# stegben/neural-locality-sensitive-hashing

Hardware: AMD Instinct MI355X
Metric: queries/sec + recall@10, SIFT1M 128-d 16-bit hash, 1/2/4/8 GPU (higher is better)
Workload: dtype f32

## Files before the change

include/nlsh_hip.h:

```cpp
#ifndef NLSH_HIP_H
#define NLSH_HIP_H

#include <stddef.h>
#include <stdint.h>

#ifdef __cplusplus
extern "C" {
#endif

#define NLSH_ABI_VERSION 4

typedef void *nlsh_stream_t;

enum {
    NLSH_OK = 0,
    NLSH_E_INVALID = -1,
    NLSH_E_UNSUPPORTED = -2,
    NLSH_E_HIP = -3,
    NLSH_E_WORKSPACE = -4
};

enum { NLSH_ACT_SIGMOID = 0, NLSH_ACT_TANH = 1 };
enum { NLSH_KEY_REF_INT16 = 0, NLSH_KEY_FULL = 1 };
enum { NLSH_METRIC_L2_EPS = 0, NLSH_METRIC_COSINE = 1, NLSH_METRIC_L2_EPS_FOLDED = 2 };
// ... 206 lines not shown
    int64_t Q;
    int32_t *qkeys, *nkeys;
    float *out_dist;
    int32_t *out_idx;
    uint64_t *out_keys;
    int32_t *out_ncand, *status;
    void *workspace;
    size_t workspace_bytes;
    int64_t max_tasks;
    nlsh_stream_t front, plan, mid, tail;
} nlsh_step_desc_t;

int nlsh_step_create(const nlsh_step_desc_t *desc, size_t desc_bytes, nlsh_step_t **step_out);
int nlsh_step_create_graph(const nlsh_step_desc_t *desc, size_t desc_bytes, nlsh_stream_t lane, nlsh_step_t **step_out);
int nlsh_step_destroy(nlsh_step_t *step);
int nlsh_step_set_weights(nlsh_step_t *step, const float *packed);
int nlsh_query_step_enqueue(nlsh_step_t *step, const float *queries, int64_t q_stride, uint64_t seed, nlsh_stream_t producer,
                            void *ev_scan_begin, void *ev_scan_end);
int nlsh_step_release(nlsh_step_t *step);
int nlsh_query_batch(const nlsh_step_desc_t *desc, size_t desc_bytes, const float *queries, int64_t q_stride, uint64_t seed,
                     int64_t row0, int lookup_done, void *ev_scan_begin, void *ev_scan_end, nlsh_stream_t stream);
int nlsh_query_batch_host(const nlsh_step_desc_t *desc, size_t desc_bytes, const float *queries, int64_t q_stride, uint64_t seed,
                          int64_t row0, int lookup_done, int32_t *host_out, size_t host_words, nlsh_stream_t stream);
size_t nlsh_query_batch_ranked_scratch(int64_t Q, int H);
int nlsh_query_batch_ranked(const nlsh_step_desc_t *desc, size_t desc_bytes, const float *queries, int64_t q_stride, int lookup_done,
                            int32_t budget, void *scratch, size_t scratch_bytes, int32_t *host_out, size_t host_words,
                            void *ev_scan_begin, void *ev_scan_end, nlsh_stream_t stream);
int nlsh_step_busy(nlsh_step_t *step);

int nlsh_merge_topk(const uint64_t *keys_in, int64_t row_stride, int G, int64_t Q, int k, const int32_t *ncand_in,
                    float *out_dist, int32_t *out_idx, int32_t *out_ncand, nlsh_stream_t stream);

#define NLSH_MAX_TABLES 16
int nlsh_merge_topk_unique(const uint64_t *keys_in, int64_t row_stride, int G, int64_t Q, int k, const int32_t *ncand_in,
                           float *out_dist, int32_t *out_idx, uint64_t *out_keys , int32_t *out_ncand, nlsh_stream_t stream);

#define NLSH_EXACT_L2 0
#define NLSH_EXACT_COSINE 1
size_t nlsh_exact_workspace(int64_t Q, int64_t N, int k, int splits);
int nlsh_exact_topk(const float *corpus, int64_t row_stride, int64_t N, int d,
                    const float *queries, int64_t q_stride, int64_t Q, int k, int metric,
                    int64_t self_row0 , int splits ,
                    float *out_dist, int32_t *out_idx, void *workspace, size_t workspace_bytes, nlsh_stream_t stream);

#ifdef __cplusplus
}
// ... 3 lines not shown
```

neural-locality-sensitive-hashing_amd/csrc/step.hip:

```cpp
#include <cstdlib>
#include <new>

#include "step_nodes.h"

#include "scan_bucket_args.h"

using namespace nlsh;

struct nlsh_step {
    EncPlan enc;
    nlsh_step_desc_t d;
    int dims[NLSH_MAX_LAYERS + 1];
    hipEvent_t ready, encoded, planned, scanned, done;
    bool done_pending;
    hipStream_t lane;
    hipGraph_t graph;
    hipGraphExec_t exec;
    hipGraphNode_t enc_node, scan_node;
    bool graph_failed;
};

static BucketScanCall step_scan_call(const nlsh_step_desc_t &d, const float *queries, int64_t q_stride, hipStream_t stream, int phases) {
    BucketScanCall c = {};
    c.corpus = d.corpus_sorted; c.row_stride = d.row_stride; c.d = d.d; c.gid = d.gid; c.uniq = d.uniq_keys; c.offsets = d.offsets;
    c.bucket_order = d.bucket_order; c.nb = d.n_buckets; c.cell_of = d.cell_of; c.cell_offsets = d.cell_offsets; c.n_cells = d.n_cells;
    c.inv_norm = d.inv_norm; c.queries = queries; c.q_stride = q_stride; c.Q = d.Q; c.qkeys = d.qkeys; c.nkeys = d.nkeys;
    c.P = d.n_probes; c.k = d.k; c.metric = d.metric; c.algo = d.algo; c.seg = d.seg_rows;
    c.out_dist = d.out_dist; c.out_idx = d.out_idx; c.out_keys = d.out_keys; c.out_ncand = d.out_ncand; c.status = d.status;
    c.workspace = d.workspace; c.workspace_bytes = d.workspace_bytes; c.max_tasks = d.max_tasks;
    c.stream = stream; c.phases = phases;
    return c;
}
constexpr int SCAN_AND_MERGE = NLSH_PHASE_SCAN | NLSH_PHASE_MERGE;
static int step_scan_check(const BucketScanCall &c) { return scan_call_check("scan_topk", c, SCAN_NEEDS_TOPK_OUT | SCAN_ALLOWS_PLAN_REST); }
static int step_scan_prepare(const BucketScanCall &c, BucketScanPrep *p) {
    const int rc = step_scan_check(c);
    return rc != NLSH_OK ? rc : bucket_scan_args(c, p);
}
static int step_scan_run(const BucketScanCall &c) {
    const int rc = step_scan_check(c);
    if (rc != NLSH_OK || c.Q == 0) return rc;
    return scan_call_run(c);
// ... 23 lines not shown
static int step_create(const nlsh_step_desc_t *desc, size_t desc_bytes, hipStream_t lane, nlsh_step_t **out) {
    NLSH_REQUIRE(desc && out, NLSH_E_INVALID, "step_create: null pointer");
    NLSH_REQUIRE(desc_bytes == sizeof(nlsh_step_desc_t), NLSH_E_INVALID, "step_create: descriptor of %zu bytes, this library's is %zu (ABI %d)",
                 desc_bytes, sizeof(nlsh_step_desc_t), NLSH_ABI_VERSION);
    if (lane == nullptr) {
        NLSH_REQUIRE(desc->front && desc->mid && desc->tail, NLSH_E_INVALID, "step_create: the front, mid and tail streams must be real streams (not the default stream)");
        NLSH_REQUIRE(desc->front != desc->mid && desc->mid != desc->tail && desc->front != desc->tail && desc->plan != desc->front && desc->plan != desc->mid &&
                         desc->plan != desc->tail,
                     NLSH_E_INVALID, "step_create: front, plan, mid and tail must be DIFFERENT streams (the stages overlap only across streams, and an event is recorded on one and waited for on the next)");
    }
    NLSH_REQUIRE(desc->n_layers >= 1 && desc->n_layers <= NLSH_MAX_LAYERS && desc->dims, NLSH_E_INVALID, "step_create: n_layers=%d", desc->n_layers);
    NLSH_REQUIRE(desc->n_probes >= 1 && desc->n_probes <= NLSH_MAX_PROBES, NLSH_E_UNSUPPORTED, "step_create: n_probes=%d not in [1,%d] (one scan call per batch)",
                 desc->n_probes, NLSH_MAX_PROBES);
    NLSH_REQUIRE(desc->Q >= 1 && desc->dims[0] == desc->d, NLSH_E_INVALID, "step_create: Q=%lld, encoder input %d vs corpus dimension %d", (long long)desc->Q,
                 desc->dims[0], desc->d);
    nlsh_step *s = new (std::nothrow) nlsh_step();
    NLSH_REQUIRE(s != nullptr, NLSH_E_INVALID, "step_create: out of host memory");
    s->d = *desc;
    for (int l = 0; l <= desc->n_layers; ++l) s->dims[l] = desc->dims[l];
    s->d.dims = s->dims;
    s->ready = s->encoded = s->planned = s->scanned = s->done = nullptr;
    s->done_pending = false;
    s->lane = lane; s->graph = nullptr; s->exec = nullptr; s->enc_node = s->scan_node = nullptr;
    s->graph_failed = getenv("NLSH_STEP_NO_GRAPH") != nullptr;
    const hipStream_t last = lane ? lane : (hipStream_t)desc->tail;
    int rc = encode_plan_fill(s->enc, desc->Q, desc->n_layers, s->dims, desc->packed, desc->act, desc->key_mode, desc->n_probes, desc->n_multi_rows, 0,
                              nullptr, nullptr, nullptr, desc->qkeys, desc->nkeys);
    if (rc == NLSH_OK) {
        const BucketScanCall c = step_scan_call(s->d, desc->corpus_sorted ? desc->corpus_sorted : (const float *)desc->workspace,
                                                desc->row_stride >= desc->d ? desc->row_stride : desc->d, last, NLSH_PHASE_SCAN);
        if (desc->algo == NLSH_SCAN_QUERY_MAJOR) {
            rc = step_scan_check(c);
            if (rc == NLSH_OK) rc = query_major_workspace(c);
        } else {
            BucketScanPrep p;
            rc = step_scan_prepare(c, &p);
            if (rc == NLSH_OK && fuses_lookup(s->d)) rc = encode_plan_fuse_lookup(s->enc, p.pa);
        }
    }
    if (rc == NLSH_OK && lane != nullptr && !(fuses_lookup(s->d) && desc->max_tasks > 0)) {
        set_error("step_create_graph: graph slots take the bucket-major schedules (algo 1, 2) on a non-empty index and task table");
        rc = NLSH_E_UNSUPPORTED;
    }
    if (rc == NLSH_OK) rc = encode_plan_prepare(s->enc);
    if (rc == NLSH_OK) rc = make_event(&s->ready);
    if (rc == NLSH_OK && !lane) rc = make_event(&s->encoded);
// ... 23 lines not shown

extern "C" int nlsh_step_destroy(nlsh_step_t *s) {
    if (!s) return NLSH_OK;
    for (hipEvent_t e : {s->ready, s->encoded, s->planned, s->scanned, s->done})
        if (e) (void)hipEventDestroy(e);
    if (s->exec) (void)hipGraphExecDestroy(s->exec);
    if (s->graph) (void)hipGraphDestroy(s->graph);
    delete s;
    return NLSH_OK;
}

extern "C" int nlsh_step_set_weights(nlsh_step_t *s, const float *packed) {
    NLSH_REQUIRE(s && packed, NLSH_E_INVALID, "step_set_weights: null pointer");
    s->enc.a.packed = packed;
    s->d.packed = packed;
    return NLSH_OK;
}


static int graph_capture(nlsh_step *s, const float *queries, int64_t q_stride, uint64_t seed) {
    NLSH_CHECK_HIP(hipStreamBeginCapture(s->lane, hipStreamCaptureModeThreadLocal));
    int plan_phase, plan_blocks;
    int rc = launch_encode(s->enc, s->d, queries, q_stride, seed, s->lane, &plan_phase, &plan_blocks);
    BucketScanCall rest = step_scan_call(s->d, queries, q_stride, s->lane, plan_phase | SCAN_AND_MERGE);
    rest.plan_blocks = plan_blocks;
    if (rc == NLSH_OK) rc = step_scan_run(rest);
    hipGraph_t g = nullptr;
    const hipError_t ce = hipStreamEndCapture(s->lane, &g);
    if (rc != NLSH_OK) {
        if (g) (void)hipGraphDestroy(g);
        return rc;
    }
    NLSH_CHECK_HIP(ce);
    s->graph = g;
    EncNode en;
    ScanNode sn;
    const BucketScanCall c = step_scan_call(s->d, queries, q_stride, s->lane, NLSH_PHASE_SCAN);
    rc = step_scan_check(c);
    if (rc == NLSH_OK) rc = bucket_scan_node(c, &sn);
    if (rc == NLSH_OK) rc = encode_plan_node(s->enc, queries, q_stride, seed, nullptr, &en);
    if (rc != NLSH_OK) return rc;
    size_t n = 0;
    NLSH_CHECK_HIP(hipGraphGetNodes(g, nullptr, &n));
    hipGraphNode_t nodes[16];
    NLSH_REQUIRE(n >= 2 && n <= 16, NLSH_E_HIP, "step graph: %zu nodes captured", n);
    NLSH_CHECK_HIP(hipGraphGetNodes(g, nodes, &n));
    for (size_t i = 0; i < n; ++i) {
        hipGraphNodeType t;
        NLSH_CHECK_HIP(hipGraphNodeGetType(nodes[i], &t));
        if (t != hipGraphNodeTypeKernel) continue;
        hipKernelNodeParams kp;
        NLSH_CHECK_HIP(hipGraphKernelNodeGetParams(nodes[i], &kp));
        if (kp.func == en.p.func) s->enc_node = nodes[i];
        else if (kp.func == sn.p.func) s->scan_node = nodes[i];
    }
    NLSH_REQUIRE(s->enc_node && s->scan_node, NLSH_E_HIP, "step graph: the encode / scan nodes were not found among the %zu captured", n);
    NLSH_CHECK_HIP(hipGraphInstantiate(&s->exec, g, nullptr, nullptr, 0));
    return NLSH_OK;
}

static int graph_enqueue(nlsh_step *s, const float *queries, int64_t q_stride, uint64_t seed, nlsh_stream_t producer, void *ev0, void *ev1) {
    const hipStream_t lane = s->lane;
    if ((hipStream_t)producer != lane) {
        const hipError_t qe = hipStreamQuery((hipStream_t)producer);
        if (qe == hipErrorNotReady) {
            (void)hipGetLastError();
            NLSH_CHECK_HIP(hipEventRecord(s->ready, (hipStream_t)producer));
            NLSH_CHECK_HIP(hipStreamWaitEvent(lane, s->ready, 0));
        } else {
            NLSH_CHECK_HIP(qe);
        }
    }
    int rc;
    if (!s->exec && !s->graph_failed && !(ev0 || ev1)) {
        if (graph_capture(s, queries, q_stride, seed) != NLSH_OK) {
            s->graph_failed = true;
            if (s->exec) { (void)hipGraphExecDestroy(s->exec); s->exec = nullptr; }
            if (s->graph) { (void)hipGraphDestroy(s->graph); s->graph = nullptr; }
            (void)hipGetLastError();
        }
    }
    if (ev0 || ev1 || !s->exec) {
        int plan_phase, plan_blocks;
        rc = launch_encode(s->enc, s->d, queries, q_stride, seed, lane, &plan_phase, &plan_blocks);
        BucketScanCall rest = step_scan_call(s->d, queries, q_stride, lane, plan_phase | SCAN_AND_MERGE);
        rest.plan_blocks = plan_blocks; rest.ev_begin = ev0; rest.ev_end = ev1;
        if (rc == NLSH_OK) rc = step_scan_run(rest);
        if (rc != NLSH_OK) return rc;
    } else {
        const BucketScanCall c = step_scan_call(s->d, queries, q_stride, lane, NLSH_PHASE_SCAN);
        BucketScanPrep p;
        EncNode en;
        ScanNode sn;
        rc = step_scan_prepare(c, &p);
        if (rc == NLSH_OK) rc = encode_plan_fuse_lookup(s->enc, p.pa);
        if (rc == NLSH_OK) rc = encode_plan_node(s->enc, queries, q_stride, seed, &p.pa, &en);
        if (rc == NLSH_OK) rc = bucket_scan_node(c, &sn);
        if (rc != NLSH_OK) return rc;
        NLSH_CHECK_HIP(hipGraphExecKernelNodeSetParams(s->exec, s->enc_node, &en.p));
        NLSH_CHECK_HIP(hipGraphExecKernelNodeSetParams(s->exec, s->scan_node, &sn.p));
        NLSH_CHECK_HIP(hipGraphLaunch(s->exec, lane));
    }
    if (s->d.hold_done) s->done_pending = true;
    else NLSH_CHECK_HIP(hipEventRecord(s->done, lane));
    return NLSH_OK;
}

extern "C" int nlsh_query_step_enqueue(nlsh_step_t *s, const float *queries, int64_t q_stride, uint64_t seed, nlsh_stream_t producer,
                                       void *ev_scan_begin, void *ev_scan_end) {
    NLSH_REQUIRE(s && queries, NLSH_E_INVALID, "query_step_enqueue: null pointer");
    NLSH_REQUIRE(!s->done_pending, NLSH_E_INVALID, "query_step_enqueue: the slot's previous batch was not released (nlsh_step_release)");
    if (s->lane) return graph_enqueue(s, queries, q_stride, seed, producer, ev_scan_begin, ev_scan_end);
    const hipStream_t front = (hipStream_t)s->d.front, mid = (hipStream_t)s->d.mid, tail = (hipStream_t)s->d.tail;
    NLSH_CHECK_HIP(hipStreamWaitEvent(front, s->done, 0));
    bool wait_producer = (hipStream_t)producer != front;
    if (wait_producer) {
        const hipError_t qe = hipStreamQuery((hipStream_t)producer);
        if (qe == hipSuccess) wait_producer = false;
        else if (qe == hipErrorNotReady) (void)hipGetLastError();
        else NLSH_CHECK_HIP(qe);
    }
    if (wait_producer) {
        NLSH_CHECK_HIP(hipEventRecord(s->ready, (hipStream_t)producer));
        NLSH_CHECK_HIP(hipStreamWaitEvent(front, s->ready, 0));
// ... 186 lines not shown
    c.ev_begin = ev_scan_begin; c.ev_end = ev_scan_end;
    BucketScanPrep p;
    int rc = step_scan_prepare(c, &p);
    if (rc != NLSH_OK) return rc;
    int plan_phase = NLSH_PHASE_PLAN, plan_blocks = 0;
    if (!lookup_done) {
        char *base = (char *)scratch;
        float *z = (float *)(base + w.z);
        uint32_t *code = (uint32_t *)(base + w.code);
        EncPlan enc;
        rc = encode_plan_fill(enc, desc->Q, desc->n_layers, desc->dims, desc->packed, desc->act, desc->key_mode, 1, desc->n_multi_rows, 0, z, nullptr, code,
                              (int32_t *)(base + w.keys), (int32_t *)(base + w.nkeys));
        if (rc == NLSH_OK) rc = encode_plan_launch(enc, queries, q_stride, 0, s);
        if (rc == NLSH_OK)
            rc = probe_ranked_plan_launch(z, H, code, H, desc->key_mode, desc->n_multi_rows, budget, p.pa, desc->qkeys, desc->nkeys, s, &plan_blocks);
        if (rc != NLSH_OK) return rc;
        plan_phase = NLSH_PHASE_PLAN_REST;
    }
    c.phases = plan_phase | SCAN_AND_MERGE;
    c.plan_blocks = plan_blocks;
    c.host_out = mapped;
    return bucket_scan_run(c);
}
```

neural-locality-sensitive-hashing_amd/nlsh_amd/_capi.py:

```python
import ctypes
import os
import subprocess

_PKG = os.path.dirname(os.path.dirname(os.path.abspath(__file__)))
LIB_PATH = os.environ.get("NLSH_HIP_LIB") or os.path.join(_PKG, "lib", "libnlsh_hip.so")
CSRC = os.path.join(_PKG, "csrc")

OK, E_INVALID, E_UNSUPPORTED, E_HIP, E_WORKSPACE = 0, -1, -2, -3, -4
ACT_SIGMOID, ACT_TANH = 0, 1
KEY_REF_INT16, KEY_FULL = 0, 1
METRIC_L2_EPS, METRIC_COSINE, METRIC_L2_EPS_FOLDED = 0, 1, 2
SCAN_QUERY_MAJOR, SCAN_BUCKET_MAJOR, SCAN_BUCKET_TILED = 0, 1, 2
STORE_F32, STORE_F16, STORE_U8 = 0, 1, 2
MAX_LAYERS, MAX_HASH_BITS, MAX_PROBES, MAX_K, MAX_DIM, MAX_WIDTH = 8, 32, 64, 64, 1024, 632
MAX_K_TILED = 256
MAX_TABLES = 16
PHASE_PLAN, PHASE_SCAN, PHASE_MERGE = 1, 2, 4
PHASE_ALL = 7
MAX_ENCODE_PROBES = 128
EXACT_L2, EXACT_COSINE = 0, 1
PROBES = ("sampled", "ranked")
PROBE_RANKED_ROWS_PER_WORKGROUP = 4
MAX_STREAM_WIDTH = 4096

SYMBOLS = (
    "nlsh_abi_version", "nlsh_last_error",
    "nlsh_encoder_packed_floats", "nlsh_encoder_pack", "nlsh_encode_hash", "nlsh_pack_codes",
    "nlsh_encoder_stream_packed_floats", "nlsh_encoder_stream_pack", "nlsh_encode_stream_workspace", "nlsh_encode_hash_stream",
    "nlsh_build_csr_workspace", "nlsh_build_csr", "nlsh_bucket_order_workspace", "nlsh_bucket_order", "nlsh_build_cells_workspace", "nlsh_build_cells", "nlsh_gather_rows",
    "nlsh_scan_workspace", "nlsh_scan_workspace_layout", "nlsh_scan_topk", "nlsh_scan_topk_phase", "nlsh_scan_topk_cells_phase",
    "nlsh_merge_topk",
    "nlsh_step_create", "nlsh_step_create_graph", "nlsh_step_destroy", "nlsh_step_set_weights", "nlsh_query_step_enqueue", "nlsh_step_release", "nlsh_step_busy", "nlsh_query_batch",
    "nlsh_query_batch_host",
    "nlsh_exact_workspace", "nlsh_exact_topk",
    "nlsh_probe_ranked", "nlsh_probe_ranked_budget",
    "nlsh_query_batch_ranked_scratch", "nlsh_query_batch_ranked",
    "nlsh_csr_update_workspace", "nlsh_csr_update",
    "nlsh_scan_topk_cells_phase_typed", "nlsh_gather_rows_typed", "nlsh_csr_update_typed",
    "nlsh_row_filter_words", "nlsh_row_filter_build", "nlsh_scan_topk_cells_phase_filtered",
    "nlsh_merge_topk_unique",
    "nlsh_range_workspace", "nlsh_range_sort_workspace", "nlsh_range_count", "nlsh_range_fill",
    "nlsh_sq8_train_workspace", "nlsh_sq8_train", "nlsh_gather_rows_sq8", "nlsh_csr_update_sq8", "nlsh_scan_topk_cells_phase_sq8",
)


class NlshHipError(RuntimeError):
    def __init__(self, code, msg):
        super().__init__(f"nlsh_hip error {code}: {msg}")
        self.code = code


_lib = None
vp, i32, i64, u64, sz = ctypes.c_void_p, ctypes.c_int, ctypes.c_int64, ctypes.c_uint64, ctypes.c_size_t


class StepDesc(ctypes.Structure):
# ... 111 lines not shown
    L.nlsh_row_filter_words.restype = sz
    L.nlsh_row_filter_words.argtypes = [i64]
    L.nlsh_row_filter_build.restype = i32
    L.nlsh_row_filter_build.argtypes = [vp, i64, vp, i64, vp, i64, ctypes.c_int32, i32, vp, vp, vp]
    L.nlsh_merge_topk.restype = i32
    L.nlsh_merge_topk.argtypes = [vp, i64, i32, i64, i32, vp, vp, vp, vp, vp]
    L.nlsh_merge_topk_unique.restype = i32
    L.nlsh_merge_topk_unique.argtypes = [vp, i64, i32, i64, i32, vp, vp, vp, vp, vp, vp]
    L.nlsh_step_create.restype = i32
    L.nlsh_step_create.argtypes = [ctypes.POINTER(StepDesc), sz, ctypes.POINTER(vp)]
    L.nlsh_step_create_graph.restype = i32
    L.nlsh_step_create_graph.argtypes = [ctypes.POINTER(StepDesc), sz, vp, ctypes.POINTER(vp)]
    for name in ("nlsh_step_destroy", "nlsh_step_release", "nlsh_step_busy"):
        getattr(L, name).restype = i32
        getattr(L, name).argtypes = [vp]
    L.nlsh_step_set_weights.restype = i32
    L.nlsh_step_set_weights.argtypes = [vp, vp]
    L.nlsh_query_step_enqueue.restype = i32
    L.nlsh_query_step_enqueue.argtypes = [vp, vp, i64, u64, vp, vp, vp]
    L.nlsh_query_batch.restype = i32
    L.nlsh_query_batch.argtypes = [ctypes.POINTER(StepDesc), sz, vp, i64, u64, i64, i32, vp, vp, vp]
    L.nlsh_query_batch_host.restype = i32
    L.nlsh_query_batch_host.argtypes = [ctypes.POINTER(StepDesc), sz, vp, i64, u64, i64, i32, vp, sz, vp]
    L.nlsh_exact_workspace.restype = sz
    L.nlsh_exact_workspace.argtypes = [i64, i64, i32, i32]
    L.nlsh_exact_topk.restype = i32
    L.nlsh_exact_topk.argtypes = [vp, i64, i64, i32, vp, i64, i64, i32, i32, i64, i32, vp, vp, vp, sz, vp]
    L.nlsh_probe_ranked.restype = i32
    L.nlsh_probe_ranked.argtypes = [vp, i64, vp, i64, i32, i32, i32, i64, vp, vp, vp, vp]
    L.nlsh_probe_ranked_budget.restype = i32
    L.nlsh_probe_ranked_budget.argtypes = [vp, i64, vp, i64, i32, i32, i32, i64, vp, vp, i32, i32, vp, vp, vp, vp, vp]
    L.nlsh_query_batch_ranked_scratch.restype = sz
    L.nlsh_query_batch_ranked_scratch.argtypes = [i64, i32]
    L.nlsh_query_batch_ranked.restype = i32
    L.nlsh_query_batch_ranked.argtypes = [ctypes.POINTER(StepDesc), sz, vp, i64, i32, ctypes.c_int32, vp, sz, vp, sz, vp, vp, vp]
    _lib = L
    return L


def check(rc):
    if rc != OK:
        raise NlshHipError(rc, lib().nlsh_last_error().decode("utf-8", "replace"))


def probe_mode(probes, default="sampled"):
    mode = default if probes is None else probes
# ... 16 lines not shown
```

neural-locality-sensitive-hashing_amd/nlsh_amd/indexer.py:

```python
import contextlib
import ctypes
import gc
import numbers
import operator
import threading
import weakref
from typing import Dict, List, Optional, Sequence, Set, Tuple

import numpy as np
import torch

from . import _capi
from .data import metric_of
from .hashings import host_key_set, keys_to_sets

HASH_BATCH = 4096


class _CollectorPause:

    def __init__(self):
        self._lock = threading.Lock()
        self._depth = 0
        self._found_enabled = False
# ... 532 lines not shown
            ids = torch.arange(self.next_id, self.next_id + M, dtype=torch.int32, device=dev)
        else:
            ids = torch.as_tensor(add_ids, device=dev)
            if ids.shape != (M,) or ids.dtype.is_floating_point or ids.dtype.is_complex or ids.dtype == torch.bool:
                raise ValueError("ids must be M integers")
            if ids.dtype != torch.int32:
                if int(ids.min().item()) < -(1 << 31) or int(ids.max().item()) > 0x7FFFFFFF:
                    raise ValueError("row ids are int32")
                ids = ids.to(torch.int32)
            ids = ids.contiguous()
            if int(torch.unique(ids).numel()) != M:
                raise ValueError("ids must be distinct")
            if bool(torch.isin(ids, self.gid).any().item()):
                raise ValueError("ids must be new: some are in the index already")
        return vectors, ids, keys

    def _drop_derived(self):
        self._cells = {}
        self._index2row = None
        self._perm_host = None
        self._e_sb = None
        self._ws = {}
        self._max_tasks = {}
        for name in ("_range_plans", "_ranked_key_tables", "_key_tables", "_held", "_bucket_dir"):
            self.__dict__.pop(name, None)

    def row_filter(self, allow=None, deny=None, mask=None) -> RowFilter:
        if (allow is not None) + (deny is not None) + (mask is not None) != 1:
            raise ValueError("row_filter takes exactly one of allow=, deny= and mask=")
        if self.metric not in ("l2", "cosine"):
            raise NotImplementedError("row filters need metric 'l2' or 'cosine': the filter is read by the tiled scan kernel")
        ids = None
        if mask is not None:
            if not isinstance(mask, torch.Tensor) or mask.dtype not in (torch.bool, torch.uint8) or mask.dim() != 1:
                raise ValueError("mask must be a 1-d bool or uint8 tensor indexed by id - id_base")
            if mask.device.type != "cuda":
                raise _capi.NlshHipError(_capi.E_INVALID, "mask must be device-resident; there is no CPU path")
        else:
            given = allow if allow is not None else deny
            name = "allow" if allow is not None else "deny"
            if isinstance(given, torch.Tensor):
                ids = given
                if ids.numel() and (ids.dtype.is_floating_point or ids.dtype.is_complex or ids.dtype == torch.bool):
                    raise ValueError(f"{name} must hold integer ids")
            else:
                arr = np.asarray(list(given))
                if arr.size and arr.dtype.kind not in "iu":
# ... 180 lines not shown

    def _tkey(self, algo, Q, P):
        return (algo, Q, P, self.choose_window(Q, P, algo))

    def _estimate_tasks(self, Q, P, seg, algo):
        biased = self._size_biased_bucket()
        if algo == _capi.SCAN_BUCKET_TILED:
            est = Q * min(P, 4) * (1.0 / 16 + biased / 256 / 16) + self.n_buckets
        elif algo == _capi.SCAN_BUCKET_MAJOR:
            est = Q * min(P, 4) * (1.0 / 4 + biased / seg / 4) + self.n_buckets
        else:
            est = Q * (1.0 + min(P, 4) * biased / seg)
        return int(min(max(1.5 * est + 1024, Q + 1024), 2 ** 31 - 8))

    def _task_table(self, algo, Q, P):
        tkey = self._tkey(algo, Q, P)
        window = tkey[3]
        max_tasks = self._max_tasks.get(tkey)
        if max_tasks is None:
            grown = [v for (a_, q_, p_, w_), v in self._max_tasks.items() if a_ == algo and q_ >= Q and p_ >= P and w_ == window]
            max_tasks = self._max_tasks[tkey] = min(grown) if grown else self._estimate_tasks(Q, P, self.seg_rows or 512, algo)
        return tkey, window, max_tasks

    def _workspace(self, dev, stream, bucket_major, ws_bytes):
        wkey = (stream, bucket_major)
        ws = self._ws.get(wkey)
        if ws is None or ws.numel() < ws_bytes or ws.device != dev:
            ws = self._ws[wkey] = torch.zeros((max(ws_bytes, 1),), dtype=torch.uint8, device=dev)
        return wkey, ws

    @staticmethod
    def _outputs(Q, k, dev, want_keys=False):
        out_dist = torch.empty((Q, k), dtype=torch.float32, device=dev)
        pack = torch.empty((Q * k + Q + 2,), dtype=torch.int32, device=dev)
        out_keys = torch.empty((Q, k), dtype=torch.int64, device=dev) if want_keys else None
        out_idx, ncand, status = pack.split((Q * k, Q, 2))
        return out_dist, pack, out_idx.view(Q, k), ncand, status, out_keys

    def _set_last(self, status, algo, window, pack, tkey, max_tasks):
        self.last_status = status
        self.last_algo, self.last_window = algo, window
        self._last_pack, self._last_tkey, self._last_max_tasks = pack, tkey, max_tasks

    def scan_tensors(self, query_vectors, keys, nkeys, k=10, want_keys=False, check=True, events=None, algo=None, filter=None):
        filter = self._checked_filter(filter, algo)
        if self.metric not in ("l2", "cosine"):
            raise NotImplementedError("fused scan needs metric 'l2' or 'cosine' (use SIFT.distance / Glove.distance)")
        q = self._as_queries(query_vectors)
# ... 406 lines not shown
            if not check:
                break
            needed, overflow = status.cpu().tolist()
            if self._settle(tkey, needed, overflow, max_tasks):
                break
            lookup_done = 1
        self._set_last(status, algo, window, pack, tkey, max_tasks)
        return out_dist, out_idx, ncand, out_keys, keys, nkeys

    def _rows_of_key(self, key):
        key = int(key)
        if self._hashing.key_mode == _capi.KEY_FULL and key >= (1 << 31):
            key -= 1 << 32
        directory = self.__dict__.get("_bucket_dir")
        if directory is None:
            directory = self._bucket_dir = dict(zip(self._uniq_host.tolist(), zip(self._offs_host[:-1].tolist(), self._offs_host[1:].tolist())))
        span = directory.get(key)
        if span is None:
            return []
        if self._perm_host is None:
            self._perm_host = self.gid.cpu().numpy().astype(np.int64)
        return self._perm_host[span[0]:span[1]].tolist()

    def _range_plan(self, q, keys, nkeys, k, lo, hi, algo, n_multi, host=None, ranked=False):
        Q_all, P = keys.shape
        dev, m = q.device, hi - lo
        stream = _stream(dev)
        ckey = (stream, Q_all, lo, hi, P, k, algo, self.l2_form, keys.data_ptr(), q.shape[1], ranked)
        plans = self.__dict__.setdefault("_range_plans", {})
        plan = plans.get(ckey)
        tkey, window, max_tasks = self._task_table(algo, m, P)
        sig = self._hashing._weights_signature()
        host_ptr = None if host is None else host.data_ptr()
        if (plan is not None and plan["max_tasks"] == max_tasks and plan["ws"] is self._ws.get(plan["wkey"]) and plan["window"] == window
                and plan["host_ptr"] == host_ptr):
            if plan["sig"] != sig:
                plan["packed"] = self._hashing.packed_weights()
                plan["desc"].packed = plan["packed"].data_ptr()
                plan["sig"] = sig
            return plan
        d = q.shape[1]
        wkey, ws = self._workspace(dev, stream, True, _capi.lib().nlsh_scan_workspace(m, P, k, max_tasks, self.n_buckets, d))
        rk, rn = keys[lo:hi], nkeys[lo:hi]
        out_dist, pack, out_idx, ncand, status, _ = self._outputs(m, k, dev)
        enc = self._hashing.ranked_encode_args(P) if ranked else self._hashing.encode_args(P, rk, rn)[0]
        scratch = self._ranked_scratch(m, dev) if ranked else None
        desc = self._step_desc(self._scan_fields(m, d, rk, rn, k, algo, max_tasks, out_dist, out_idx, None, ncand, status, ws, window),
                               enc, min(max(n_multi - lo, 0), m))
        plan = plans[ckey] = dict(desc=desc, ref=ctypes.byref(desc), size=ctypes.sizeof(desc), dims_arr=enc[1], packed=self._hashing.packed_weights(), sig=sig,
                                  keys=rk, nkeys=rn, out_dist=out_dist, pack=pack, status=status, ws=ws, wkey=wkey, max_tasks=max_tasks, tkey=tkey,
                                  window=window, stream=stream, host_ptr=host_ptr, host_words=0 if host is None else host.numel(),
                                  scratch=scratch, scratch_ptr=None if scratch is None else scratch.data_ptr(),
                                  scratch_bytes=0 if scratch is None else scratch.numel())
        if len(plans) > 64:
            for old_key in list(plans)[:-32]:
                del plans[old_key]
        return plan

    def _host_form(self, k, fused):
        return fused is not None and k <= _capi.MAX_K

    def _range_tensors(self, q, keys, nkeys, k, lo, hi, algo, fused, host=None):
        if fused is None:
            if hi - lo == q.shape[0]:
                self.scan_tensors(q, keys, nkeys, k=k, check=False, algo=algo)
# ... 43 lines not shown
                self._range_tensors(q, keys, nkeys, k, 0, Q, algo, fused)
                to_ids, to_keys, to_nkeys, _ = pin.split((n, Q * P, Q, pin.numel() - words))
                to_ids.copy_(self._last_pack, non_blocking=True)
                if self.compat:
                    to_keys.view(Q, P).copy_(keys, non_blocking=True)
                    to_nkeys.copy_(nkeys, non_blocking=True)
            self._release_held()
            if queued is not None:
                queued()
                queued = None
            torch.cuda.current_stream(q.device).synchronize()
            host = pin.numpy()
            if self._settle(self._last_tkey, int(host[n - 2]), int(host[n - 1]) if Q else 0, self._last_max_tasks):
                return self._block_views(host, Q, k, P, host_form)

    query_chunks = None
    _CHUNK_MIN_ROWS = 2048

    def _n_chunks(self):
        if self.query_chunks is not None:
            return int(self.query_chunks)
        return 1 if self.defer_result_release else 2

    def _chunked_results(self, q, keys, nkeys, k, n_chunks, fused=None, queued=None):
        Q, P = keys.shape
        algo = self.choose_algo(Q, P)
        stream = torch.cuda.current_stream(q.device)
        bounds = [(Q * c // n_chunks, Q * (c + 1) // n_chunks) for c in range(n_chunks)]
        per = max(hi - lo for lo, hi in bounds)
        words = (per * k + per + 2 + per * P + per + 3) // 4 * 4
        if self._pin is None or self._pin.numel() < n_chunks * words:
            self._pin = torch.empty((max(n_chunks * words, 1 << 16),), dtype=torch.int32, pin_memory=True)
        pin = self._pin
        host_form = self._host_form(k, fused)

        def launch(c, lo, hi):
            m = hi - lo
            n = m * k + m + 2
            block = pin[c * words:c * words + n + m * P + m]
            if host_form and m:
                self._range_tensors(q, keys, nkeys, k, lo, hi, algo, fused, block)
            else:
                self._range_tensors(q, keys, nkeys, k, lo, hi, algo, fused)
                to_ids, to_keys, to_nkeys = block.split((n, m * P, m))
                to_ids.copy_(self._last_pack, non_blocking=True)
                if self.compat:
                    to_keys.view(m, P).copy_(keys[lo:hi], non_blocking=True)
                    to_nkeys.copy_(nkeys[lo:hi], non_blocking=True)
            ev = torch.cuda.Event()
            ev.record(stream)
            return ev, self._last_tkey, self._last_max_tasks

        inflight = [launch(c, lo, hi) for c, (lo, hi) in enumerate(bounds)]
        self._release_held()
        if queued is not None:
            queued()
        host = pin.numpy()
        for c, (lo, hi) in enumerate(bounds):
            m = hi - lo
            a = host[c * words:(c + 1) * words]
            n = m * k + m + 2
            while True:
                ev, tkey, max_tasks = inflight[c]
                ev.synchronize()
                if self._settle(tkey, int(a[n - 2]), int(a[n - 1]) if m else 0, max_tasks):
                    break
                inflight[c] = launch(c, lo, hi)
            yield (lo, hi) + self._block_views(a, m, k, P, host_form and m > 0)

    promote_results = False
    defer_result_release = False
    untracked_results = False
    _FULL_COLLECT_EVERY = 2048
    _promotions = 0

    @classmethod
    def _plain_lists(cls, idx_h, nc_h):
        promote = _collector_pause.application_state() and cls.promote_results and len(nc_h) >= 512 and gc.get_freeze_count() == 0
        if promote:
            gc.collect(0)
        with _collector_pause:
            if _rows_to_lists is not None and idx_h.dtype == np.int32 and idx_h.ndim == 2 and idx_h.flags.c_contiguous:
                out = _rows_to_lists(idx_h, idx_h.shape[0], idx_h.shape[1], bool(cls.untracked_results)), nc_h.tolist()
            else:
                out = idx_h.tolist(), nc_h.tolist()
            if promote:
                gc.freeze()
                gc.unfreeze()
                Indexer._promotions += 1
                if Indexer._promotions % cls._FULL_COLLECT_EVERY == 0:
                    gc.collect()
# ... 193 lines not shown
```

Measured before the change: 9.789 million.

## Add range sets to run chunk front stages concurrently on prioritized lanes

Adds a native range-set object that creates one step per query chunk, each on its own stream (the first with higher priority). The encode/plan front stage of later chunks runs in a captured graph on its own lane, while their scan and merge are serialized back onto the first lane and write results straight into mapped host blocks. The Python chunked path uses this set instead of launching chunks one after another, so chunk fronts overlap and per-chunk launch overhead drops. This adds several streams and events plus cached per-lane workspaces, and brings more complex retry and error paths.

```diff
diff --git a/include/nlsh_hip.h b/include/nlsh_hip.h
--- a/include/nlsh_hip.h
+++ b/include/nlsh_hip.h
@@ -252,6 +252,16 @@
                      int64_t row0, int lookup_done, void *ev_scan_begin, void *ev_scan_end, nlsh_stream_t stream);
 int nlsh_query_batch_host(const nlsh_step_desc_t *desc, size_t desc_bytes, const float *queries, int64_t q_stride, uint64_t seed,
                           int64_t row0, int lookup_done, int32_t *host_out, size_t host_words, nlsh_stream_t stream);
+#define NLSH_MAX_RANGES 8
+typedef struct nlsh_range_set nlsh_range_set_t;
+int nlsh_range_set_create(int n_ranges, const nlsh_step_desc_t *const *descs, size_t desc_bytes, const int64_t *row0,
+                          int32_t *const *host_out, const size_t *host_words, const nlsh_stream_t *lanes ,
+                          nlsh_range_set_t **set_out);
+int nlsh_range_set_enqueue(nlsh_range_set_t *set, const float *queries, int64_t q_stride, uint64_t seed, nlsh_stream_t producer);
+int nlsh_range_set_wait(nlsh_range_set_t *set, int range);
+int nlsh_range_set_set_weights(nlsh_range_set_t *set, const float *packed);
+int nlsh_range_set_info(const nlsh_range_set_t *set, int *n_graphs , int *priority_levels );
+int nlsh_range_set_destroy(nlsh_range_set_t *set);
 size_t nlsh_query_batch_ranked_scratch(int64_t Q, int H);
 int nlsh_query_batch_ranked(const nlsh_step_desc_t *desc, size_t desc_bytes, const float *queries, int64_t q_stride, int lookup_done,
                             int32_t budget, void *scratch, size_t scratch_bytes, int32_t *host_out, size_t host_words,
diff --git a/neural-locality-sensitive-hashing_amd/csrc/step.hip b/neural-locality-sensitive-hashing_amd/csrc/step.hip
--- a/neural-locality-sensitive-hashing_amd/csrc/step.hip
+++ b/neural-locality-sensitive-hashing_amd/csrc/step.hip
@@ -18,6 +18,8 @@
     hipGraphExec_t exec;
     hipGraphNode_t enc_node, scan_node;
     bool graph_failed;
+    int32_t *host_mapped;
+    bool front_only;
 };
 
 static BucketScanCall step_scan_call(const nlsh_step_desc_t &d, const float *queries, int64_t q_stride, hipStream_t stream, int phases) {
@@ -87,6 +89,8 @@
     s->ready = s->encoded = s->planned = s->scanned = s->done = nullptr;
     s->done_pending = false;
     s->lane = lane; s->graph = nullptr; s->exec = nullptr; s->enc_node = s->scan_node = nullptr;
+    s->host_mapped = nullptr;
+    s->front_only = false;
     s->graph_failed = getenv("NLSH_STEP_NO_GRAPH") != nullptr;
     const hipStream_t last = lane ? lane : (hipStream_t)desc->tail;
     int rc = encode_plan_fill(s->enc, desc->Q, desc->n_layers, s->dims, desc->packed, desc->act, desc->key_mode, desc->n_probes, desc->n_multi_rows, 0,
@@ -156,8 +160,8 @@
     NLSH_CHECK_HIP(hipStreamBeginCapture(s->lane, hipStreamCaptureModeThreadLocal));
     int plan_phase, plan_blocks;
     int rc = launch_encode(s->enc, s->d, queries, q_stride, seed, s->lane, &plan_phase, &plan_blocks);
-    BucketScanCall rest = step_scan_call(s->d, queries, q_stride, s->lane, plan_phase | SCAN_AND_MERGE);
-    rest.plan_blocks = plan_blocks;
+    BucketScanCall rest = step_scan_call(s->d, queries, q_stride, s->lane, s->front_only ? plan_phase : (plan_phase | SCAN_AND_MERGE));
+    rest.plan_blocks = plan_blocks; rest.host_out = s->host_mapped;
     if (rc == NLSH_OK) rc = step_scan_run(rest);
     hipGraph_t g = nullptr;
     const hipError_t ce = hipStreamEndCapture(s->lane, &g);
@@ -188,9 +192,53 @@
         if (kp.func == en.p.func) s->enc_node = nodes[i];
         else if (kp.func == sn.p.func) s->scan_node = nodes[i];
     }
-    NLSH_REQUIRE(s->enc_node && s->scan_node, NLSH_E_HIP, "step graph: the encode / scan nodes were not found among the %zu captured", n);
+    NLSH_REQUIRE(s->enc_node && (s->scan_node || s->front_only), NLSH_E_HIP, "step graph: the encode / scan nodes were not found among the %zu captured", n);
     NLSH_CHECK_HIP(hipGraphInstantiate(&s->exec, g, nullptr, nullptr, 0));
     return NLSH_OK;
+}
+
+static void graph_ensure(nlsh_step *s, const float *queries, int64_t q_stride, uint64_t seed) {
+    if (s->exec || s->graph_failed) return;
+    if (graph_capture(s, queries, q_stride, seed) != NLSH_OK) {
+        s->graph_failed = true;
+        if (s->exec) { (void)hipGraphExecDestroy(s->exec); s->exec = nullptr; }
+        if (s->graph) { (void)hipGraphDestroy(s->graph); s->graph = nullptr; }
+        (void)hipGetLastError();
+    }
+}
+
+static int graph_nodes(nlsh_step *s, const float *queries, int64_t q_stride, uint64_t seed, EncNode *en, ScanNode *sn) {
+    const BucketScanCall c = step_scan_call(s->d, queries, q_stride, s->lane, NLSH_PHASE_SCAN);
+    BucketScanPrep p;
+    int rc = step_scan_prepare(c, &p);
+    if (rc == NLSH_OK) rc = encode_plan_fuse_lookup(s->enc, p.pa);
+    if (rc == NLSH_OK) rc = encode_plan_node(s->enc, queries, q_stride, seed, &p.pa, en);
+    if (rc == NLSH_OK) rc = bucket_scan_node(c, sn);
+    return rc;
+}
+
+static int graph_replay(nlsh_step *s, EncNode *en, ScanNode *sn) {
+    NLSH_CHECK_HIP(hipGraphExecKernelNodeSetParams(s->exec, s->enc_node, &en->p));
+    if (!s->front_only) NLSH_CHECK_HIP(hipGraphExecKernelNodeSetParams(s->exec, s->scan_node, &sn->p));
+    NLSH_CHECK_HIP(hipGraphLaunch(s->exec, s->lane));
+    return NLSH_OK;
+}
+
+static int lane_eager(nlsh_step *s, const float *queries, int64_t q_stride, uint64_t seed, void *ev0, void *ev1) {
+    int plan_phase, plan_blocks;
+    int rc = launch_encode(s->enc, s->d, queries, q_stride, seed, s->lane, &plan_phase, &plan_blocks);
+    BucketScanCall rest = step_scan_call(s->d, queries, q_stride, s->lane, s->front_only ? plan_phase : (plan_phase | SCAN_AND_MERGE));
+    rest.plan_blocks = plan_blocks; rest.ev_begin = ev0; rest.ev_end = ev1; rest.host_out = s->host_mapped;
+    if (rc == NLSH_OK) rc = step_scan_run(rest);
+    return rc;
+}
+
+static int lane_back(nlsh_step *s, const float *queries, int64_t q_stride, hipStream_t main) {
+    NLSH_CHECK_HIP(hipEventRecord(s->ready, s->lane));
+    NLSH_CHECK_HIP(hipStreamWaitEvent(main, s->ready, 0));
+    BucketScanCall back = step_scan_call(s->d, queries, q_stride, main, SCAN_AND_MERGE);
+    back.host_out = s->host_mapped;
+    return step_scan_run(back);
 }
 
 static int graph_enqueue(nlsh_step *s, const float *queries, int64_t q_stride, uint64_t seed, nlsh_stream_t producer, void *ev0, void *ev1) {
@@ -206,34 +254,16 @@
         }
     }
     int rc;
-    if (!s->exec && !s->graph_failed && !(ev0 || ev1)) {
-        if (graph_capture(s, queries, q_stride, seed) != NLSH_OK) {
-            s->graph_failed = true;
-            if (s->exec) { (void)hipGraphExecDestroy(s->exec); s->exec = nullptr; }
-            if (s->graph) { (void)hipGraphDestroy(s->graph); s->graph = nullptr; }
-            (void)hipGetLastError();
-        }
-    }
+    if (!(ev0 || ev1)) graph_ensure(s, queries, q_stride, seed);
     if (ev0 || ev1 || !s->exec) {
-        int plan_phase, plan_blocks;
-        rc = launch_encode(s->enc, s->d, queries, q_stride, seed, lane, &plan_phase, &plan_blocks);
-        BucketScanCall rest = step_scan_call(s->d, queries, q_stride, lane, plan_phase | SCAN_AND_MERGE);
-        rest.plan_blocks = plan_blocks; rest.ev_begin = ev0; rest.ev_end = ev1;
-        if (rc == NLSH_OK) rc = step_scan_run(rest);
+        rc = lane_eager(s, queries, q_stride, seed, ev0, ev1);
         if (rc != NLSH_OK) return rc;
     } else {
-        const BucketScanCall c = step_scan_call(s->d, queries, q_stride, lane, NLSH_PHASE_SCAN);
-        BucketScanPrep p;
         EncNode en;
         ScanNode sn;
-        rc = step_scan_prepare(c, &p);
-        if (rc == NLSH_OK) rc = encode_plan_fuse_lookup(s->enc, p.pa);
-        if (rc == NLSH_OK) rc = encode_plan_node(s->enc, queries, q_stride, seed, &p.pa, &en);
-        if (rc == NLSH_OK) rc = bucket_scan_node(c, &sn);
+        rc = graph_nodes(s, queries, q_stride, seed, &en, &sn);
+        if (rc == NLSH_OK) rc = graph_replay(s, &en, &sn);
         if (rc != NLSH_OK) return rc;
-        NLSH_CHECK_HIP(hipGraphExecKernelNodeSetParams(s->exec, s->enc_node, &en.p));
-        NLSH_CHECK_HIP(hipGraphExecKernelNodeSetParams(s->exec, s->scan_node, &sn.p));
-        NLSH_CHECK_HIP(hipGraphLaunch(s->exec, lane));
     }
     if (s->d.hold_done) s->done_pending = true;
     else NLSH_CHECK_HIP(hipEventRecord(s->done, lane));
@@ -466,3 +496,166 @@
     c.host_out = mapped;
     return bucket_scan_run(c);
 }
+
+struct nlsh_range_set {
+    int n;
+    nlsh_step *range[NLSH_MAX_RANGES];
+    hipStream_t lane[NLSH_MAX_RANGES];
+    bool owns_lanes;
+    int priority_levels;
+    int64_t row0[NLSH_MAX_RANGES];
+    const int32_t *host_out[NLSH_MAX_RANGES];
+    size_t need[NLSH_MAX_RANGES];
+    hipEvent_t ready;
+    EncNode en[NLSH_MAX_RANGES];
+    ScanNode sn[NLSH_MAX_RANGES];
+};
+
+extern "C" int nlsh_range_set_destroy(nlsh_range_set_t *set) {
+    if (!set) return NLSH_OK;
+    for (int i = 0; i < set->n; ++i) {
+        if (set->lane[i]) (void)hipStreamSynchronize(set->lane[i]);
+        (void)nlsh_step_destroy(set->range[i]);
+        if (set->owns_lanes && set->lane[i]) (void)hipStreamDestroy(set->lane[i]);
+    }
+    if (set->ready) (void)hipEventDestroy(set->ready);
+    delete set;
+    return NLSH_OK;
+}
+
+extern "C" int nlsh_range_set_create(int n_ranges, const nlsh_step_desc_t *const *descs, size_t desc_bytes, const int64_t *row0,
+                                     int32_t *const *host_out, const size_t *host_words, const nlsh_stream_t *lanes, nlsh_range_set_t **out) {
+    NLSH_REQUIRE(out, NLSH_E_INVALID, "range_set_create: null pointer");
+    *out = nullptr;
+    NLSH_REQUIRE(descs && row0 && host_out && host_words, NLSH_E_INVALID, "range_set_create: null pointer");
+    NLSH_REQUIRE(desc_bytes == sizeof(nlsh_step_desc_t), NLSH_E_INVALID, "range_set_create: descriptor of %zu bytes, this library's is %zu (ABI %d)",
+                 desc_bytes, sizeof(nlsh_step_desc_t), NLSH_ABI_VERSION);
+    NLSH_REQUIRE(n_ranges >= 2 && n_ranges <= NLSH_MAX_RANGES, NLSH_E_INVALID, "range_set_create: n_ranges=%d not in [2,%d]", n_ranges, NLSH_MAX_RANGES);
+    size_t need[NLSH_MAX_RANGES];
+    for (int i = 0; i < n_ranges; ++i) {
+        const nlsh_step_desc_t *d = descs[i];
+        NLSH_REQUIRE(d, NLSH_E_INVALID, "range_set_create: descriptor %d is null", i);
+        NLSH_REQUIRE(d->Q >= 1 && d->Q < (1ll << 31) && row0[i] >= 0, NLSH_E_INVALID, "range_set_create: range %d: Q=%lld, row0=%lld", i, (long long)d->Q,
+                     (long long)row0[i]);
+        NLSH_REQUIRE(d->k >= 1 && d->k <= NLSH_MAX_K, NLSH_E_INVALID, "range_set_create: range %d: k=%d not in [1,%d] (the host-writing merge)", i, d->k, NLSH_MAX_K);
+        NLSH_REQUIRE(d->algo == NLSH_SCAN_BUCKET_MAJOR || d->algo == NLSH_SCAN_BUCKET_TILED, NLSH_E_INVALID,
+                     "range_set_create: range %d: algo=%d: only the bucket-major schedules (1, 2) have a host-writing merge", i, d->algo);
+        NLSH_REQUIRE(d->n_probes >= 1 && d->n_probes <= NLSH_MAX_PROBES, NLSH_E_UNSUPPORTED, "range_set_create: range %d: n_probes=%d not in [1,%d]", i,
+                     d->n_probes, NLSH_MAX_PROBES);
+        need[i] = (size_t)d->Q * (size_t)(d->k + 1 + d->n_probes + 1) + 2;
+        NLSH_REQUIRE(host_out[i], NLSH_E_INVALID, "range_set_create: range %d: host_out is null", i);
+        NLSH_REQUIRE(host_words[i] >= need[i], NLSH_E_INVALID, "range_set_create: range %d: host_out of %zu words, Q=%lld k=%d n_probes=%d need %zu", i,
+                     host_words[i], (long long)d->Q, d->k, d->n_probes, need[i]);
+        for (int j = 0; j < i; ++j) {
+            NLSH_REQUIRE(d->workspace != descs[j]->workspace && d->status != descs[j]->status && d->qkeys != descs[j]->qkeys && d->nkeys != descs[j]->nkeys &&
+                             host_out[i] != host_out[j],
+                         NLSH_E_INVALID, "range_set_create: ranges %d and %d share a workspace, status words, key table rows or host block (they run concurrently)", j, i);
+            NLSH_REQUIRE(!lanes || lanes[i] != lanes[j], NLSH_E_INVALID, "range_set_create: ranges %d and %d were given the same lane (a lane orders ONE range)", j, i);
+        }
+        NLSH_REQUIRE(!lanes || lanes[i] != nullptr, NLSH_E_INVALID, "range_set_create: lane %d must be a real stream (not the default stream: it is captured)", i);
+    }
+    int32_t *mapped[NLSH_MAX_RANGES];
+    for (int i = 0; i < n_ranges; ++i)
+        if (const int mrc = host_block_mapped("range_set_create", host_out[i], need[i], &mapped[i])) return mrc;
+    nlsh_range_set *set = new (std::nothrow) nlsh_range_set();
+    NLSH_REQUIRE(set != nullptr, NLSH_E_INVALID, "range_set_create: out of host memory");
+    set->n = 0; set->owns_lanes = lanes == nullptr; set->priority_levels = 0; set->ready = nullptr;
+    for (int i = 0; i < NLSH_MAX_RANGES; ++i) { set->range[i] = nullptr; set->lane[i] = nullptr; }
+    int rc = NLSH_OK, least = 0, greatest = 0;
+    if (set->owns_lanes) {
+        if (hipDeviceGetStreamPriorityRange(&least, &greatest) != hipSuccess) { (void)hipGetLastError(); least = greatest = 0; }
+        set->priority_levels = least == greatest ? 1 : (least > greatest ? least - greatest : greatest - least) + 1;
+    }
+    for (int i = 0; i < n_ranges && rc == NLSH_OK; ++i) {
+        set->n = i + 1;
+        if (set->owns_lanes) {
+            if (hipStreamCreateWithPriority(&set->lane[i], hipStreamNonBlocking, i == 0 ? greatest : least) != hipSuccess) {
+                set_error("range_set_create: hipStreamCreateWithPriority failed");
+                set->lane[i] = nullptr;
+                rc = NLSH_E_HIP;
+                break;
+            }
+        } else {
+            set->lane[i] = (hipStream_t)lanes[i];
+        }
+        rc = step_create(descs[i], desc_bytes, set->lane[i], &set->range[i]);
+        if (rc != NLSH_OK) break;
+        set->range[i]->d.hold_done = 0;
+        set->range[i]->host_mapped = mapped[i];
+        set->range[i]->front_only = i > 0;
+        if (i == 0) set->range[i]->graph_failed = true;
+        set->range[i]->enc.a.row0 = row0[i];
+        set->row0[i] = row0[i]; set->host_out[i] = host_out[i]; set->need[i] = need[i];
+    }
+    if (rc == NLSH_OK) rc = make_event(&set->ready);
+    if (rc != NLSH_OK) {
+        (void)nlsh_range_set_destroy(set);
+        return rc;
+    }
+    *out = set;
+    return NLSH_OK;
+}
+
+extern "C" int nlsh_range_set_set_weights(nlsh_range_set_t *set, const float *packed) {
+    NLSH_REQUIRE(set && packed, NLSH_E_INVALID, "range_set_set_weights: null pointer");
+    for (int i = 0; i < set->n; ++i) (void)nlsh_step_set_weights(set->range[i], packed);
+    return NLSH_OK;
+}
+
+extern "C" int nlsh_range_set_info(const nlsh_range_set_t *set, int *n_graphs, int *priority_levels) {
+    NLSH_REQUIRE(set, NLSH_E_INVALID, "range_set_info: null pointer");
+    int g = 0;
+    for (int i = 0; i < set->n; ++i) g += set->range[i]->exec != nullptr;
+    if (n_graphs) *n_graphs = g;
+    if (priority_levels) *priority_levels = set->priority_levels;
+    return NLSH_OK;
+}
+
+extern "C" int nlsh_range_set_enqueue(nlsh_range_set_t *set, const float *queries, int64_t q_stride, uint64_t seed, nlsh_stream_t producer) {
+    NLSH_REQUIRE(set && queries, NLSH_E_INVALID, "range_set_enqueue: null pointer");
+    NLSH_REQUIRE(q_stride >= set->range[0]->d.d, NLSH_E_INVALID, "range_set_enqueue: q_stride=%lld < d=%d", (long long)q_stride, set->range[0]->d.d);
+    for (int i = 0; i < set->n; ++i) {
+        int32_t *mapped = nullptr;
+        if (const int mrc = host_block_mapped("range_set_enqueue", set->host_out[i], set->need[i], &mapped)) return mrc;
+        NLSH_REQUIRE(mapped == set->range[i]->host_mapped, NLSH_E_INVALID, "range_set_enqueue: range %d: the host block is mapped elsewhere than at create", i);
+    }
+    for (int i = 0; i < set->n; ++i) {
+        nlsh_step *s = set->range[i];
+        const float *q = queries + set->row0[i] * q_stride;
+        graph_ensure(s, q, q_stride, seed);
+        if (s->exec) {
+            const int rc = graph_nodes(s, q, q_stride, seed, &set->en[i], &set->sn[i]);
+            if (rc != NLSH_OK) return rc;
+        } else {
+            BucketScanPrep p;
+            const int rc = step_scan_prepare(step_scan_call(s->d, q, q_stride, s->lane, NLSH_PHASE_PLAN_REST | SCAN_AND_MERGE), &p);
+            if (rc != NLSH_OK) return rc;
+        }
+    }
+    bool wait_producer = false;
+    const hipError_t qe = hipStreamQuery((hipStream_t)producer);
+    if (qe == hipErrorNotReady) {
+        (void)hipGetLastError();
+        NLSH_CHECK_HIP(hipEventRecord(set->ready, (hipStream_t)producer));
+        wait_producer = true;
+    } else {
+        NLSH_CHECK_HIP(qe);
+    }
+    for (int i = 0; i < set->n; ++i) {
+        nlsh_step *s = set->range[i];
+        if (wait_producer) NLSH_CHECK_HIP(hipStreamWaitEvent(s->lane, set->ready, 0));
+        if (i > 0) NLSH_CHECK_HIP(hipStreamWaitEvent(s->lane, s->done, 0));
+        const float *q = queries + set->row0[i] * q_stride;
+        int rc = s->exec ? graph_replay(s, &set->en[i], &set->sn[i]) : lane_eager(s, q, q_stride, seed, nullptr, nullptr);
+        if (rc == NLSH_OK && i > 0) rc = lane_back(s, q, q_stride, set->lane[0]);
+        if (rc != NLSH_OK) return rc;
+        NLSH_CHECK_HIP(hipEventRecord(s->done, set->lane[0]));
+    }
+    return NLSH_OK;
+}
+
+extern "C" int nlsh_range_set_wait(nlsh_range_set_t *set, int i) {
+    NLSH_REQUIRE(set && i >= 0 && i < set->n, NLSH_E_INVALID, "range_set_wait: range %d of a set of %d", i, set ? set->n : 0);
+    NLSH_CHECK_HIP(hipEventSynchronize(set->range[i]->done));
+    return NLSH_OK;
+}
diff --git a/neural-locality-sensitive-hashing_amd/nlsh_amd/_capi.py b/neural-locality-sensitive-hashing_amd/nlsh_amd/_capi.py
--- a/neural-locality-sensitive-hashing_amd/nlsh_amd/_capi.py
+++ b/neural-locality-sensitive-hashing_amd/nlsh_amd/_capi.py
@@ -14,6 +14,7 @@
 STORE_F32, STORE_F16, STORE_U8 = 0, 1, 2
 MAX_LAYERS, MAX_HASH_BITS, MAX_PROBES, MAX_K, MAX_DIM, MAX_WIDTH = 8, 32, 64, 64, 1024, 632
 MAX_K_TILED = 256
+MAX_RANGES = 8
 MAX_TABLES = 16
 PHASE_PLAN, PHASE_SCAN, PHASE_MERGE = 1, 2, 4
 PHASE_ALL = 7
@@ -32,6 +33,7 @@
     "nlsh_merge_topk",
     "nlsh_step_create", "nlsh_step_create_graph", "nlsh_step_destroy", "nlsh_step_set_weights", "nlsh_query_step_enqueue", "nlsh_step_release", "nlsh_step_busy", "nlsh_query_batch",
     "nlsh_query_batch_host",
+    "nlsh_range_set_create", "nlsh_range_set_enqueue", "nlsh_range_set_wait", "nlsh_range_set_set_weights", "nlsh_range_set_info", "nlsh_range_set_destroy",
     "nlsh_exact_workspace", "nlsh_exact_topk",
     "nlsh_probe_ranked", "nlsh_probe_ranked_budget",
     "nlsh_query_batch_ranked_scratch", "nlsh_query_batch_ranked",
@@ -189,6 +191,18 @@
     L.nlsh_query_batch.argtypes = [ctypes.POINTER(StepDesc), sz, vp, i64, u64, i64, i32, vp, vp, vp]
     L.nlsh_query_batch_host.restype = i32
     L.nlsh_query_batch_host.argtypes = [ctypes.POINTER(StepDesc), sz, vp, i64, u64, i64, i32, vp, sz, vp]
+    L.nlsh_range_set_create.restype = i32
+    L.nlsh_range_set_create.argtypes = [i32, vp, sz, vp, vp, vp, vp, ctypes.POINTER(vp)]
+    L.nlsh_range_set_enqueue.restype = i32
+    L.nlsh_range_set_enqueue.argtypes = [vp, vp, i64, u64, vp]
+    L.nlsh_range_set_wait.restype = i32
+    L.nlsh_range_set_wait.argtypes = [vp, i32]
+    L.nlsh_range_set_set_weights.restype = i32
+    L.nlsh_range_set_set_weights.argtypes = [vp, vp]
+    L.nlsh_range_set_info.restype = i32
+    L.nlsh_range_set_info.argtypes = [vp, ctypes.POINTER(i32), ctypes.POINTER(i32)]
+    L.nlsh_range_set_destroy.restype = i32
+    L.nlsh_range_set_destroy.argtypes = [vp]
     L.nlsh_exact_workspace.restype = sz
     L.nlsh_exact_workspace.argtypes = [i64, i64, i32, i32]
     L.nlsh_exact_topk.restype = i32
diff --git a/neural-locality-sensitive-hashing_amd/nlsh_amd/indexer.py b/neural-locality-sensitive-hashing_amd/nlsh_amd/indexer.py
--- a/neural-locality-sensitive-hashing_amd/nlsh_amd/indexer.py
+++ b/neural-locality-sensitive-hashing_amd/nlsh_amd/indexer.py
@@ -578,7 +578,7 @@
         self._e_sb = None
         self._ws = {}
         self._max_tasks = {}
-        for name in ("_range_plans", "_ranked_key_tables", "_key_tables", "_held", "_bucket_dir"):
+        for name in ("_range_sets", "_range_plans", "_ranked_key_tables", "_key_tables", "_held", "_bucket_dir"):
             self.__dict__.pop(name, None)
 
     def row_filter(self, allow=None, deny=None, mask=None) -> RowFilter:
@@ -805,8 +805,8 @@
             max_tasks = self._max_tasks[tkey] = min(grown) if grown else self._estimate_tasks(Q, P, self.seg_rows or 512, algo)
         return tkey, window, max_tasks
 
-    def _workspace(self, dev, stream, bucket_major, ws_bytes):
-        wkey = (stream, bucket_major)
+    def _workspace(self, dev, stream, bucket_major, ws_bytes, lane=0):
+        wkey = (stream, bucket_major) if not lane else ((stream, lane), bucket_major)
         ws = self._ws.get(wkey)
         if ws is None or ws.numel() < ws_bytes or ws.device != dev:
             ws = self._ws[wkey] = torch.zeros((max(ws_bytes, 1),), dtype=torch.uint8, device=dev)
@@ -1259,11 +1259,11 @@
             self._perm_host = self.gid.cpu().numpy().astype(np.int64)
         return self._perm_host[span[0]:span[1]].tolist()
 
-    def _range_plan(self, q, keys, nkeys, k, lo, hi, algo, n_multi, host=None, ranked=False):
+    def _range_plan(self, q, keys, nkeys, k, lo, hi, algo, n_multi, host=None, ranked=False, lane=0):
         Q_all, P = keys.shape
         dev, m = q.device, hi - lo
         stream = _stream(dev)
-        ckey = (stream, Q_all, lo, hi, P, k, algo, self.l2_form, keys.data_ptr(), q.shape[1], ranked)
+        ckey = (stream, Q_all, lo, hi, P, k, algo, self.l2_form, keys.data_ptr(), q.shape[1], ranked, lane)
         plans = self.__dict__.setdefault("_range_plans", {})
         plan = plans.get(ckey)
         tkey, window, max_tasks = self._task_table(algo, m, P)
@@ -1277,7 +1277,7 @@
                 plan["sig"] = sig
             return plan
         d = q.shape[1]
-        wkey, ws = self._workspace(dev, stream, True, _capi.lib().nlsh_scan_workspace(m, P, k, max_tasks, self.n_buckets, d))
+        wkey, ws = self._workspace(dev, stream, True, _capi.lib().nlsh_scan_workspace(m, P, k, max_tasks, self.n_buckets, d), lane)
         rk, rn = keys[lo:hi], nkeys[lo:hi]
         out_dist, pack, out_idx, ncand, status, _ = self._outputs(m, k, dev)
         enc = self._hashing.ranked_encode_args(P) if ranked else self._hashing.encode_args(P, rk, rn)[0]
@@ -1367,6 +1367,65 @@
             return int(self.query_chunks)
         return 1 if self.defer_result_release else 2
 
+    class _RangeSet:
+        __slots__ = ("handle", "plans", "sig", "block_step")
+
+        def __init__(self, plans, bounds):
+            n = len(plans)
+            descs = (ctypes.c_void_p * n)(*[ctypes.addressof(p["desc"]) for p in plans])
+            row0 = (ctypes.c_int64 * n)(*[lo for lo, _ in bounds])
+            blocks = (ctypes.c_void_p * n)(*[p["host_ptr"] for p in plans])
+            words = (ctypes.c_size_t * n)(*[p["host_words"] for p in plans])
+            handle = ctypes.c_void_p()
+            self.handle, self.plans, self.sig, self.block_step = None, plans, plans[0]["sig"], 0
+            _capi.check(_capi.lib().nlsh_range_set_create(n, descs, plans[0]["size"], row0, blocks, words, None, ctypes.byref(handle)))
+            self.handle = handle
+
+        def info(self):
+            graphs, levels = ctypes.c_int(0), ctypes.c_int(0)
+            _capi.check(_capi.lib().nlsh_range_set_info(self.handle, ctypes.byref(graphs), ctypes.byref(levels)))
+            return graphs.value, levels.value
+
+        def __del__(self):
+            handle, self.handle = self.handle, None
+            if handle:
+                try:
+                    _capi.lib().nlsh_range_set_destroy(handle)
+                except Exception:
+                    pass
+
+    def _range_set(self, q, keys, nkeys, k, bounds, algo, n_multi, blocks):
+        P = keys.shape[1]
+        stream = _stream(q.device)
+        sets = self.__dict__.setdefault("_range_sets", {})
+        skey = (stream, keys.shape, k, algo, self.l2_form, keys.data_ptr(), q.shape[1], len(bounds))
+        rs = sets.get(skey)
+        sig = self._hashing._weights_signature()
+        if rs is not None and rs.sig == sig:
+            mt, ws, base, step = self._max_tasks, self._ws, self._pin.data_ptr(), rs.block_step
+            for c, plan in enumerate(rs.plans):
+                if (mt.get(plan["tkey"]) != plan["max_tasks"] or plan["ws"] is not ws.get(plan["wkey"]) or plan["host_ptr"] != base + c * step
+                        or plan["window"] != self.choose_window(plan["desc"].Q, P, algo)):
+                    break
+            else:
+                return rs
+        plans = [self._range_plan(q, keys, nkeys, k, lo, hi, algo, n_multi, blocks(c), lane=c) for c, (lo, hi) in enumerate(bounds)]
+        if rs is None or any(a is not b for a, b in zip(rs.plans, plans)):
+            sets.pop(skey, None)
+            rs = None
+            if len(sets) > 8:
+                sets.clear()
+            rs = sets[skey] = self._RangeSet(plans, bounds)
+            rs.block_step = plans[1]["host_ptr"] - plans[0]["host_ptr"]
+        if rs.sig != plans[0]["sig"]:
+            _capi.check(_capi.lib().nlsh_range_set_set_weights(rs.handle, plans[0]["packed"].data_ptr()))
+            rs.sig = plans[0]["sig"]
+        return rs
+
+    @staticmethod
+    def _range_wait(rs, c):
+        _capi.check(_capi.lib().nlsh_range_set_wait(rs.handle, c))
+
     def _chunked_results(self, q, keys, nkeys, k, n_chunks, fused=None, queued=None):
         Q, P = keys.shape
         algo = self.choose_algo(Q, P)
@@ -1379,11 +1438,25 @@
         pin = self._pin
         host_form = self._host_form(k, fused)
 
-        def launch(c, lo, hi):
+        def blocks(c):
+            return pin[c * words:c * words + (bounds[c][1] - bounds[c][0]) * (k + 1 + P + 1) + 2]
+        as_set = (host_form and fused[0] != "ranked" and 1 < n_chunks <= _capi.MAX_RANGES and min(hi - lo for lo, hi in bounds) > 0)
+
+        def launch(c, lo, hi, lookup_done=0):
             m = hi - lo
             n = m * k + m + 2
-            block = pin[c * words:c * words + n + m * P + m]
-            if host_form and m:
+            block = blocks(c)
+            if lookup_done:
+                plan = self._range_plan(q, keys, nkeys, k, lo, hi, algo, fused[2], block, lane=c)
+                try:
+                    _capi.check(_capi.lib().nlsh_query_batch_host(plan["ref"], plan["size"], q[lo:hi].data_ptr(), q.stride(0), fused[1], lo, 1,
+                                                                  plan["host_ptr"], plan["host_words"], plan["stream"]))
+                except _capi.NlshHipError:
+                    self._ws.pop(plan["wkey"], None)
+                    self._range_plans.clear()
+                    raise
+                self._set_last(plan["status"], algo, plan["window"], plan["pack"], plan["tkey"], plan["max_tasks"])
+            elif host_form and m:
                 self._range_tensors(q, keys, nkeys, k, lo, hi, algo, fused, block)
             else:
                 self._range_tensors(q, keys, nkeys, k, lo, hi, algo, fused)
@@ -1396,22 +1469,46 @@
             ev.record(stream)
             return ev, self._last_tkey, self._last_max_tasks
 
-        inflight = [launch(c, lo, hi) for c, (lo, hi) in enumerate(bounds)]
-        self._release_held()
-        if queued is not None:
-            queued()
-        host = pin.numpy()
-        for c, (lo, hi) in enumerate(bounds):
-            m = hi - lo
-            a = host[c * words:(c + 1) * words]
-            n = m * k + m + 2
-            while True:
-                ev, tkey, max_tasks = inflight[c]
-                ev.synchronize()
-                if self._settle(tkey, int(a[n - 2]), int(a[n - 1]) if m else 0, max_tasks):
-                    break
-                inflight[c] = launch(c, lo, hi)
-            yield (lo, hi) + self._block_views(a, m, k, P, host_form and m > 0)
+        rs, waited = None, 0
+        if as_set:
+            rs = self._range_set(q, keys, nkeys, k, bounds, algo, fused[2], blocks)
+            try:
+                _capi.check(_capi.lib().nlsh_range_set_enqueue(rs.handle, q.data_ptr(), q.stride(0), fused[1], rs.plans[0]["stream"]))
+            except _capi.NlshHipError:
+                for plan in rs.plans:
+                    self._ws.pop(plan["wkey"], None)
+                self._range_plans.clear()
+                self.__dict__.pop("_range_sets", None)
+                raise
+            last = rs.plans[-1]
+            self._set_last(last["status"], algo, last["window"], last["pack"], last["tkey"], last["max_tasks"])
+            inflight = [(None, plan["tkey"], plan["max_tasks"]) for plan in rs.plans]
+        else:
+            inflight = [launch(c, lo, hi) for c, (lo, hi) in enumerate(bounds)]
+        try:
+            self._release_held()
+            if queued is not None:
+                queued()
+            host = pin.numpy()
+            for c, (lo, hi) in enumerate(bounds):
+                m = hi - lo
+                a = host[c * words:(c + 1) * words]
+                n = m * k + m + 2
+                while True:
+                    ev, tkey, max_tasks = inflight[c]
+                    if ev is None:
+                        self._range_wait(rs, c)
+                        waited = c + 1
+                    else:
+                        ev.synchronize()
+                    if self._settle(tkey, int(a[n - 2]), int(a[n - 1]) if m else 0, max_tasks):
+                        break
+                    inflight[c] = launch(c, lo, hi, lookup_done=1 if as_set else 0)
+                yield (lo, hi) + self._block_views(a, m, k, P, host_form and m > 0)
+        finally:
+            if rs is not None:
+                for c in range(waited, len(bounds)):
+                    self._range_wait(rs, c)
 
     promote_results = False
     defer_result_release = False
```

Result: no change. 9.679 million (median of 2 runs) (-1.1%).
